# SYSTRAN/faster-whisper

Hardware: AMD Instinct MI355X
Metric: audio-sec/sec (RTF) large-v3 fp16 beam=5 batch=16 (higher is better)
Workload: dtype f16

## Files before the change

### faster_whisper_amd/csrc/attn_enc.hip

```cpp
#include "common.h"
#include "kernels.h"

#define AE_Q 128
#define AE_KV 64
#define AE_VSTRIDE 68
#define AE_LAG 5.0f

__global__ __launch_bounds__(256) void attn_enc_kernel(const half_t* __restrict__ q, const half_t* __restrict__ k,
                                                       int64_t ld, int64_t qk_bstride,
                                                       const half_t* __restrict__ vt, int64_t ldvt,
                                                       int64_t vt_bstride, half_t* __restrict__ out, int64_t ldo,
                                                       int64_t o_bstride, int T, int H, int n_pairs, int n_qt,
                                                       int order) {
  __shared__ __attribute__((aligned(16))) half_t sK[2][AE_KV * 64];
  __shared__ __attribute__((aligned(16))) half_t sV[2][64 * AE_VSTRIDE];

  const int tid = threadIdx.x, lane = tid & 63, wave = tid >> 6;
  const int hi = lane >> 5, l31 = lane & 31;
  const int xcd = blockIdx.x & 7, idx = blockIdx.x >> 3;
  const int pair = order ? (int)blockIdx.x / n_qt : (idx / n_qt) * 8 + xcd;
  if (pair >= n_pairs) return;
  const int b = pair / H, h = pair - b * H, q0 = (order ? (int)blockIdx.x % n_qt : idx % n_qt) * AE_Q;

  const half_t* qb = q + (size_t)b * qk_bstride + h * 64;
  const half_t* kb = k + (size_t)b * qk_bstride + h * 64;
  const half_t* vb = vt + (size_t)b * vt_bstride + (size_t)(h * 64) * ldvt;

  half8_t qf[4];
  {
    int qr = q0 + wave * 32 + l31;
    if (qr > T - 1) qr = T - 1;
    const half_t* qp = qb + (size_t)qr * ld + hi * 8;
#pragma unroll
    for (int ks = 0; ks < 4; ++ks) {
      half8_t v = *reinterpret_cast<const half8_t*>(qp + ks * 16);
#pragma unroll
      for (int e = 0; e < 8; ++e) v[e] = (half_t)((float)v[e] * (0.125f * 1.4426950408889634f));
      qf[ks] = v;
    }
  }

  const int c = tid & 7, r0 = tid >> 3;
  const int nkt = (T + AE_KV - 1) / AE_KV;
  intx4 rk[2], rv[2];
  auto gload = [&](int kt) {
#pragma unroll
    for (int i = 0; i < 2; ++i) {
      const int row = r0 + 32 * i;
      int key = kt * AE_KV + row;
      if (key > T - 1) key = T - 1;
      rk[i] = *reinterpret_cast<const intx4*>(kb + (size_t)key * ld + c * 8);
      rv[i] = *reinterpret_cast<const intx4*>(vb + (size_t)row * ldvt + kt * AE_KV + c * 8);
    }
  };
  auto lstore = [&](int buf) {
#pragma unroll
    for (int i = 0; i < 2; ++i) {
      const int row = r0 + 32 * i;
      *reinterpret_cast<intx4*>(&sK[buf][row * 64 + ((c ^ ((row >> 1) & 7)) << 3)]) = rk[i];
      intx2* dv = reinterpret_cast<intx2*>(&sV[buf][row * AE_VSTRIDE + c * 8]);
      dv[0] = intx2{rv[i][0], rv[i][1]};
      dv[1] = intx2{rv[i][2], rv[i][3]};
    }
  };

  gload(0);
  lstore(0);
  __syncthreads();

  floatx16 o[2] = {floatx16{0}, floatx16{0}};
  floatx16 lsum = floatx16{0};
  const half8_t ones8 = {(half_t)1.f, (half_t)1.f, (half_t)1.f, (half_t)1.f, (half_t)1.f, (half_t)1.f, (half_t)1.f, (half_t)1.f};
  float m_ref = 0.f;
  floatx16 cneg = floatx16{0};

  for (int kt = 0; kt < nkt; ++kt) {
    const int cur = kt & 1;
    const bool more = (kt + 1) < nkt;
    if (more) gload(kt + 1);

    floatx16 s[2];
#pragma unroll
    for (int ks = 0; ks < 4; ++ks) {
      const int chunk = ks * 2 + hi;
#pragma unroll
      for (int kb2 = 0; kb2 < 2; ++kb2) {
        const int row = kb2 * 32 + l31;
        const half8_t kf = *reinterpret_cast<const half8_t*>(&sK[cur][row * 64 + ((chunk ^ ((row >> 1) & 7)) << 3)]);
        s[kb2] = __builtin_amdgcn_mfma_f32_32x32x16_f16(kf, qf[ks], ks == 0 ? cneg : s[kb2], 0, 0, 0);
      }
    }
    const int kbase = kt * AE_KV + 4 * hi;
    const bool tail = (kt * AE_KV + AE_KV) > T;
    if (tail) {
#pragma unroll
      for (int kb2 = 0; kb2 < 2; ++kb2)
#pragma unroll
        for (int r = 0; r < 16; ++r) {
          const int key = kbase + kb2 * 32 + (r & 3) + 8 * (r >> 2);
          if (key >= T) s[kb2][r] = -1.0e30f;
        }
    }
    float mx = fmaxf(s[0][0], s[1][0]);
#pragma unroll
    for (int r = 1; r < 16; ++r) mx = __builtin_fmaxf(__builtin_fmaxf(mx, s[0][r]), s[1][r]);
    mx = pair32_max(mx);
    if (kt == 0 || __builtin_amdgcn_ballot_w64(mx > AE_LAG) != 0) {
      const float delta = kt == 0 ? mx : fmaxf(mx, 0.f);
      const float alpha = kt == 0 ? 1.f : __builtin_amdgcn_exp2f(-delta);
      m_ref += delta;
#pragma unroll
      for (int r = 0; r < 16; ++r) { cneg[r] = -m_ref; lsum[r] *= alpha; }
#pragma unroll
      for (int dt = 0; dt < 2; ++dt)
#pragma unroll
        for (int r = 0; r < 16; ++r) o[dt][r] *= alpha;
#pragma unroll
      for (int kb2 = 0; kb2 < 2; ++kb2)
#pragma unroll
        for (int r = 0; r < 16; ++r) s[kb2][r] -= delta;
    }
#pragma unroll
    for (int kb2 = 0; kb2 < 2; ++kb2)
#pragma unroll
      for (int r = 0; r < 16; ++r) s[kb2][r] = __builtin_amdgcn_exp2f(s[kb2][r]);

#pragma unroll
    for (int kb2 = 0; kb2 < 2; ++kb2)
#pragma unroll
      for (int ks2 = 0; ks2 < 2; ++ks2) {
        half8_t pf;
#pragma unroll
        for (int e = 0; e < 8; e += 2) {
          const half2_t h2 = {(half_t)s[kb2][ks2 * 8 + e], (half_t)s[kb2][ks2 * 8 + e + 1]};
          pf[e] = h2[0]; pf[e + 1] = h2[1];
        }
        lsum = __builtin_amdgcn_mfma_f32_32x32x16_f16(ones8, pf, lsum, 0, 0, 0);
        const int koff = kb2 * 32 + ks2 * 16 + 4 * hi;
#pragma unroll
        for (int dt = 0; dt < 2; ++dt) {
          const half_t* vr = &sV[cur][(dt * 32 + l31) * AE_VSTRIDE + koff];
          const half4_t v0 = *reinterpret_cast<const half4_t*>(vr);
          const half4_t v1 = *reinterpret_cast<const half4_t*>(vr + 8);
          half8_t vf;
#pragma unroll
          for (int e = 0; e < 4; ++e) { vf[e] = v0[e]; vf[4 + e] = v1[e]; }
          o[dt] = __builtin_amdgcn_mfma_f32_32x32x16_f16(vf, pf, o[dt], 0, 0, 0);
        }
      }

    if (more) lstore(cur ^ 1);
    __syncthreads();
  }

  const float inv = 1.0f / lsum[0];
  const int qr = q0 + wave * 32 + l31;
  if (qr < T) {
    half_t* op = out + (size_t)b * o_bstride + (size_t)qr * ldo + h * 64;
#pragma unroll
    for (int dt = 0; dt < 2; ++dt)
#pragma unroll
      for (int g = 0; g < 4; ++g) {
        half4_t ov;
#pragma unroll
        for (int e = 0; e < 4; ++e) ov[e] = (half_t)(o[dt][g * 4 + e] * inv);
        *reinterpret_cast<half4_t*>(op + dt * 32 + 8 * g + 4 * hi) = ov;
      }
  }
}

namespace fwk {
void launch_attn_enc(hipStream_t st, const half_t* q, const half_t* k, int64_t ld, int64_t qk_bstride,
                     const half_t* vt, int64_t ldvt, int64_t vt_bstride, half_t* out, int64_t ldo,
                     int64_t o_bstride, int B, int H, int T, int order) {
  const int n_qt = (T + AE_Q - 1) / AE_Q, n_pairs = B * H;
  const int grid = ((n_pairs + 7) / 8) * 8 * n_qt;
  attn_enc_kernel<<<grid, 256, 0, st>>>(q, k, ld, qk_bstride, vt, ldvt, vt_bstride, out, ldo, o_bstride, T, H, n_pairs, n_qt, order);
}
}
```

### faster_whisper_amd/csrc/engine.hip

```cpp
#include "engine.h"

#include <math.h>
#include <stdarg.h>
#include <stdio.h>
#include <stdlib.h>
#include <string.h>

#include <algorithm>

#include "dec_kernels.h"
#include "kernels.h"

namespace fw {

static thread_local char g_err[1024] = "";
void set_error(const char* fmt, ...) {
  va_list ap;
  va_start(ap, fmt);
  vsnprintf(g_err, sizeof(g_err), fmt, ap);
  va_end(ap);
}

int dev_alloc(void** p, size_t bytes) {
  if (bytes == 0) bytes = 256;
// ... 1499 lines not shown
  {
    std::lock_guard<std::mutex> lk(fm->impl.prof_mu);
    for (auto& p : fm->impl.prof) p = ProfAcc();
  }
  for (Model* l : fm->impl.xlanes) {
    if (!l) continue;
    prof_collect(l);
    std::lock_guard<std::mutex> lk(l->prof_mu);
    for (auto& p : l->prof) p = ProfAcc();
  }
}
int32_t fw_prof_count(void) { return PF_COUNT; }
const char* fw_prof_name(int32_t i) { return (i >= 0 && i < PF_COUNT) ? kProfNames[i] : ""; }
int32_t fw_prof_get(fw_model* fm, int32_t i, double* ms, int64_t* launches, double* flops, double* bytes) {
  FW_CHECK_ARG(fm && i >= 0 && i < PF_COUNT, "bad profile index");
  prof_collect(&fm->impl);
  ProfAcc p;
  {
    std::lock_guard<std::mutex> lk(fm->impl.prof_mu);
    p = fm->impl.prof[i];
  }
  for (Model* l : fm->impl.xlanes) {
    if (!l) continue;
    prof_collect(l);
    std::lock_guard<std::mutex> lk(l->prof_mu);
    p.ms += l->prof[i].ms; p.launches += l->prof[i].launches; p.flops += l->prof[i].flops; p.bytes += l->prof[i].bytes;
  }
  if (ms) *ms = p.ms;
  if (launches) *launches = p.launches;
  if (flops) *flops = p.flops;
  if (bytes) *bytes = p.bytes;
  return FW_OK;
}
int32_t fw_synchronize(fw_model* fm) {
  FW_CHECK_ARG(fm, "null model");
  FW_HIP(hipSetDevice(fm->impl.device));
  FW_HIP(hipStreamSynchronize(fm->impl.stream));
  if (fm->impl.dec_stream) FW_HIP(hipStreamSynchronize(fm->impl.dec_stream));
  for (Model* l : fm->impl.xlanes)
    if (l && l->dec_stream) FW_HIP(hipStreamSynchronize(l->dec_stream));
  return FW_OK;
}
int32_t fw_dev_alloc(fw_model* fm, int64_t bytes, void** out_dev) {
  FW_CHECK_ARG(fm && out_dev && bytes >= 0, "bad argument");
  FW_HIP(hipSetDevice(fm->impl.device));
  return dev_alloc(out_dev, (size_t)bytes);
}
int32_t fw_dev_free(fw_model* fm, void* dev) {
  FW_CHECK_ARG(fm, "null model");
  FW_HIP(hipSetDevice(fm->impl.device));
  if (dev) FW_HIP(hipFree(dev));
  return FW_OK;
}
int32_t fw_dev_upload(fw_model* fm, void* dst_dev, const void* src_host, int64_t bytes) {
  FW_CHECK_ARG(fm && dst_dev && src_host && bytes >= 0, "bad argument");
  FW_HIP(hipSetDevice(fm->impl.device));
  FW_HIP(hipMemcpy(dst_dev, src_host, (size_t)bytes, hipMemcpyHostToDevice));
  return FW_OK;
}

static int upload_f16(Model* m, const float* src, size_t n, half_t** dst) {
  int rc = dev_alloc_t(dst, n);
  if (rc) return rc;
  std::vector<uint16_t> tmp(n);
  for (size_t i = 0; i < n; ++i) tmp[i] = f32_to_f16_bits(src[i]);
  FW_HIP(hipMemcpy(*dst, tmp.data(), n * 2, hipMemcpyHostToDevice));
  return FW_OK;
}
static int download_f16(Model* m, const half_t* src, size_t n, float* dst) {
  std::vector<uint16_t> tmp(n);
  FW_HIP(hipStreamSynchronize(m->stream));
  FW_HIP(hipMemcpy(tmp.data(), src, n * 2, hipMemcpyDeviceToHost));
  for (size_t i = 0; i < n; ++i) {
    half_t h;
    memcpy(&h, &tmp[i], 2);
    dst[i] = (float)h;
  }
  return FW_OK;
}

static inline size_t cross_kv_frag_pos(bool vt, int kvp, int mm, int n) {
  const int c = n & 63, r = mm & 31;
  const size_t head = (size_t)(n >> 6) * kvp * 64;
  return vt ? head + ((size_t)((mm >> 5) * 4 + (c >> 4)) * 64 + ((mm >> 3) & 3) * 16 + (c & 15)) * 8 + (mm & 7)
            : head + ((size_t)((mm >> 5) * 4 + 2 * ((r >> 2) & 1) + (c >> 5)) * 64 + ((c >> 3) & 3) * 16 + (((r >> 3) << 2) | (r & 3))) * 8 + (c & 7);
}

int32_t fw_test_gemm(fw_model* fm, const float* A, const float* W, const float* bias, const float* residual,
                     int32_t M, int32_t N, int32_t K, int32_t act_gelu, int32_t use_int8, float* out) {
  FW_CHECK_ARG(fm && A && W && out, "null argument");
  Model* m = &fm->impl;
  std::lock_guard<std::mutex> lk(m->mu);
  FW_HIP(hipSetDevice(m->device));
  half_t *dA = nullptr, *dW = nullptr, *dB = nullptr, *dR = nullptr, *dC = nullptr;
  int rc;
  if ((rc = upload_f16(m, A, (size_t)M * K, &dA))) return rc;
  if ((rc = upload_f16(m, W, (size_t)N * K, &dW))) return rc;
  if (bias && (rc = upload_f16(m, bias, N, &dB))) return rc;
  if (residual && (rc = upload_f16(m, residual, (size_t)M * N, &dR))) return rc;
  if ((rc = dev_alloc_t(&dC, (size_t)M * N))) return rc;
  LinearW L{dW, dB, nullptr, nullptr, nullptr, nullptr, N, K};
  int8_t* dWq = nullptr;
  float* dWs = nullptr;
  if (use_int8) {
    if (m->compute_type != FW_COMPUTE_INT8_FLOAT16 || (int64_t)M * K > (int64_t)m->max_batch * 1500 * 4 * m->cfg.d_model ||
        M > m->max_batch * 1500) {
      set_error("int8 gemm test needs an int8_float16 model and M*K within its quantisation workspace");
      return FW_EINVAL;
    }
    std::vector<int8_t> wq((size_t)N * K);
    std::vector<float> ws(N);
    for (int n = 0; n < N; ++n) {
      float amax = 0.f;
      for (int k = 0; k < K; ++k) amax = std::max(amax, fabsf(f16_bits_to_f32(f32_to_f16_bits(W[(size_t)n * K + k]))));
      const float sc = amax > 0.f ? 127.0f / amax : 0.f;
      for (int k = 0; k < K; ++k)
        wq[(size_t)n * K + k] = (int8_t)lrintf(f16_bits_to_f32(f32_to_f16_bits(W[(size_t)n * K + k])) * sc);
      ws[n] = amax > 0.f ? amax / 127.0f : 1.0f;
    }
    if ((rc = dev_alloc_t(&dWq, wq.size()))) return rc;
    if ((rc = dev_alloc_t(&dWs, ws.size()))) return rc;
    FW_HIP(hipMemcpy(dWq, wq.data(), wq.size(), hipMemcpyHostToDevice));
    FW_HIP(hipMemcpy(dWs, ws.data(), ws.size() * sizeof(float), hipMemcpyHostToDevice));
    L.wq = dWq; L.wscale = dWs;
    if (act_gelu >= 2)
      rc = run_linear_i8(m, L, dA, nullptr, dC, M, 0, nullptr, 0, 0, M, 1, act_gelu - 2, true, 0);
    else
      rc = run_linear_i8(m, L, dA, nullptr, dC, N, 0, dR, N, 0, M, 1, act_gelu, false, 0);
  } else if (act_gelu == 8 || act_gelu == 9) {
    const bool vt = act_gelu == 9;
    if (N % 64 || residual) { set_error("fragment-major gemm test: N %% 64 == 0, no residual"); return FW_EINVAL; }
    const int kvp = (M + 31) / 32 * 32, H = N / 64;
    half_t* dF = nullptr;
    if ((rc = dev_alloc_t(&dF, (size_t)H * kvp * 64))) return rc;
    FW_HIP(hipMemset(dF, 0, (size_t)H * kvp * 64 * sizeof(half_t)));
    rc = vt ? run_linear(m, L, dA, K, 0, dF, kvp, 0, nullptr, 0, 0, M, 1, 0, true, kvp)
            : run_linear(m, L, dA, K, 0, dF, N, 0, nullptr, 0, 0, M, 1, 0, false, kvp);
    std::vector<float> hf((size_t)H * kvp * 64);
    if (!rc) rc = download_f16(m, dF, hf.size(), hf.data());
    (void)hipFree(dF);
    if (!rc) {
      for (int mm = 0; mm < kvp && !rc; ++mm)
        for (int n = 0; n < N; ++n) {
          const size_t off = cross_kv_frag_pos(vt, kvp, mm, n);
          if (mm < M) out[(size_t)mm * N + n] = hf[off];
          else if (hf[off] != 0.f) { set_error("fragment-major epilogue wrote the padded key %d", mm); rc = FW_ERUNTIME; break; }
        }
    }
    for (half_t* p : {dA, dW, dB, dR, dC})
      if (p) (void)hipFree(p);
    return rc;
  } else if (act_gelu >= 2) {
    rc = run_linear(m, L, dA, K, 0, dC, M, 0, nullptr, 0, 0, M, 1, act_gelu - 2, true);
  } else {
    rc = run_linear(m, L, dA, K, 0, dC, N, 0, dR, N, 0, M, 1, act_gelu, false);
  }
  if (!rc) rc = download_f16(m, dC, (size_t)M * N, out);
  for (half_t* p : {dA, dW, dB, dR, dC})
    if (p) (void)hipFree(p);
  if (dWq) (void)hipFree(dWq);
  if (dWs) (void)hipFree(dWs);
  return rc;
}

static inline size_t frag_pos(int64_t row, int64_t k, int64_t K, int KE) {
  const int OCT = KE / 4;
  return (size_t)((((row >> 4) * (K / KE) + k / KE) * 64 + ((k / OCT) & 3) * 16 + (row & 15)) * OCT + (k % OCT));
}

int32_t fw_test_dec_linear(fw_model* fm, const float* x, const float* W, const float* bias, const float* ln_g,
                           const float* ln_b, const float* res, int32_t R, int32_t N, int32_t K, int32_t act,
                           int32_t use_int8, float* out, float* out_from_frag) {
  FW_CHECK_ARG(fm && x && W && out && out_from_frag, "null argument");
  FW_CHECK_ARG(R >= 1 && N % 32 == 0 && K % 64 == 0, "need R >= 1, N %% 32 == 0, K %% 64 == 0");
  FW_CHECK_ARG((ln_g == nullptr) == (ln_b == nullptr), "ln_g and ln_b go together");
  Model* m = &fm->impl;
  std::lock_guard<std::mutex> lk(m->mu);
  FW_HIP(hipSetDevice(m->device));
  hipStream_t st = m->stream;
  const int R16 = (R + 15) / 16 * 16;
  auto h = [](float v) { return f16_bits_to_f32(f32_to_f16_bits(v)); };
  std::vector<void*> owned;
  auto up = [&](const void* src, size_t bytes, void** dst) -> int {
    int rc = dev_alloc(dst, bytes);
    if (rc) return rc;
    owned.push_back(*dst);
    FW_HIP(hipMemcpy(*dst, src, bytes, hipMemcpyHostToDevice));
    return FW_OK;
  };
  auto cleanup = [&]() { for (void* p : owned) (void)hipFree(p); };
  int rc = FW_OK;
  half_t *d_res = nullptr, *d_bias = nullptr, *d_out = nullptr, *d_of = nullptr;
  std::vector<uint16_t> tmp;
  if (res) {
    tmp.resize((size_t)R * N);
    for (size_t i = 0; i < tmp.size(); ++i) tmp[i] = f32_to_f16_bits(res[i]);
    if ((rc = up(tmp.data(), tmp.size() * 2, (void**)&d_res))) { cleanup(); return rc; }
  }
  if ((rc = dev_alloc_t(&d_out, (size_t)R * N))) { cleanup(); return rc; }
  owned.push_back(d_out);
  if ((rc = dev_alloc_t(&d_of, (size_t)R16 * N))) { cleanup(); return rc; }
  owned.push_back(d_of);
  FW_HIP(hipMemset(d_of, 0, (size_t)R16 * N * 2));
  if (use_int8 == 1) {
    if (m->compute_type != FW_COMPUTE_INT8_FLOAT16 || ln_g) {
      cleanup();
      set_error("int8 decoder-linear test needs an int8_float16 model and no LayerNorm");
      return FW_EINVAL;
    }
    std::vector<int8_t> wq((size_t)N * K);
    std::vector<float> ws(N);
    for (int n = 0; n < N; ++n) {
      float amax = 0.f;
      for (int k = 0; k < K; ++k) amax = std::max(amax, fabsf(h(W[(size_t)n * K + k])));
      const float sc = amax > 0.f ? 127.0f / amax : 0.f;
      for (int k = 0; k < K; ++k) wq[frag_pos(n, k, K, 64)] = (int8_t)lrintf(h(W[(size_t)n * K + k]) * sc);
      ws[n] = amax > 0.f ? amax / 127.0f : 1.0f;
    }
    int8_t *d_wq = nullptr, *d_xq = nullptr;
    float *d_ws = nullptr, *d_xs = nullptr;
    half_t* d_x = nullptr;
    tmp.resize((size_t)R * K);
    for (size_t i = 0; i < tmp.size(); ++i) tmp[i] = f32_to_f16_bits(x[i]);
    if ((rc = up(wq.data(), wq.size(), (void**)&d_wq)) || (rc = up(ws.data(), ws.size() * 4, (void**)&d_ws)) ||
        (rc = up(tmp.data(), tmp.size() * 2, (void**)&d_x))) { cleanup(); return rc; }
    if (bias) {
      tmp.resize(N);
      for (int n = 0; n < N; ++n) tmp[n] = f32_to_f16_bits(bias[n]);
      if ((rc = up(tmp.data(), (size_t)N * 2, (void**)&d_bias))) { cleanup(); return rc; }
    }
    if ((rc = dev_alloc_t(&d_xq, (size_t)R16 * K))) { cleanup(); return rc; }
    owned.push_back(d_xq);
    if ((rc = dev_alloc_t(&d_xs, (size_t)R16))) { cleanup(); return rc; }
    owned.push_back(d_xs);
    FW_HIP(hipMemset(d_xq, 0, (size_t)R16 * K));
    fwk::launch_quant_rows(st, d_x, K, nullptr, nullptr, d_xq, d_xs, R, K, 1);
    if (fwd::launch_dec_gemm_frag_i8(st, d_xq, d_xs, d_wq, d_ws, d_bias, d_res, N, d_out, N, R, N, K, act) != 0) {
      cleanup();
      set_error("int8 decoder linear: unsupported shape R=%d N=%d K=%d", R, N, K);
      return FW_ERUNTIME;
    }
    rc = download_f16(m, d_out, (size_t)R * N, out);
    if (!rc) memcpy(out_from_frag, out, (size_t)R * N * sizeof(float));
    cleanup();
    return rc;
  }
  std::vector<uint16_t> wf((size_t)N * K), xf((size_t)R16 * K, 0);
  std::vector<float> s1(N, 0.f), cf(N, 0.f);
  for (int n = 0; n < N; ++n) {
    double a1 = 0.0, ac = 0.0;
    for (int k = 0; k < K; ++k) {
      const float wv = h(W[(size_t)n * K + k]);
      const uint16_t wg = ln_g ? f32_to_f16_bits(wv * h(ln_g[k])) : f32_to_f16_bits(wv);
      wf[frag_pos(n, k, K, 32)] = wg;
      a1 += (double)f16_bits_to_f32(wg);
      if (ln_g) ac += (double)wv * (double)h(ln_b[k]);
    }
    if (bias) ac += (double)h(bias[n]);
    s1[n] = (float)a1;
    cf[n] = (float)ac;
  }
  for (int r = 0; r < R; ++r)
    for (int k = 0; k < K; ++k) xf[frag_pos(r, k, K, 32)] = f32_to_f16_bits(x[(size_t)r * K + k]);
  half_t *d_wf = nullptr, *d_xf = nullptr;
  float *d_s1 = nullptr, *d_cf = nullptr;
  if ((rc = up(wf.data(), wf.size() * 2, (void**)&d_wf)) || (rc = up(xf.data(), xf.size() * 2, (void**)&d_xf))) {
    cleanup();
    return rc;
  }
  if (ln_g) {
    if ((rc = up(s1.data(), (size_t)N * 4, (void**)&d_s1)) || (rc = up(cf.data(), (size_t)N * 4, (void**)&d_cf))) {
      cleanup();
      return rc;
    }
  } else if (bias) {
    tmp.resize(N);
    for (int n = 0; n < N; ++n) tmp[n] = f32_to_f16_bits(bias[n]);
    if ((rc = up(tmp.data(), (size_t)N * 2, (void**)&d_bias))) { cleanup(); return rc; }
  }
  const int lr =
      use_int8 >= 10 ? fwd::launch_dec_gemm_big(st, use_int8 - 10, d_xf, d_wf, d_bias, d_s1, d_cf, d_res, N, d_out, N, d_of, R, N, K, act)
      : use_int8 == 5 ? fwd::launch_dec_gemm_skinny(st, d_xf, d_wf, d_bias, d_s1, d_cf, d_res, N, d_out, N, d_of, R, N, K, act)
      : (use_int8 == 6 || use_int8 == 7) ? fwd::launch_dec_gemm_skinny_tiles(st, use_int8 - 5, d_xf, d_wf, d_bias, d_s1, d_cf, d_res, N, d_out, N, d_of, R, N, K, act)
                      : fwd::launch_dec_gemm_frag(st, d_xf, d_wf, d_bias, d_s1, d_cf, d_res, N, d_out, N, d_of, R, N, K, act);
  if (lr != 0) {
    cleanup();
    set_error("decoder linear: unsupported shape R=%d N=%d K=%d", R, N, K);
    return FW_ERUNTIME;
  }
  rc = download_f16(m, d_out, (size_t)R * N, out);
  std::vector<float> of((size_t)R16 * N);
  if (!rc) rc = download_f16(m, d_of, (size_t)R16 * N, of.data());
  if (!rc)
    for (int r = 0; r < R; ++r)
      for (int n = 0; n < N; ++n) out_from_frag[(size_t)r * N + n] = of[frag_pos(r, n, N, 32)];
  cleanup();
  return rc;
}

int32_t fw_dec_big_min_rows(void) { return fwd::dec_big_min_rows(); }
int32_t fw_dec_big_min_rows_of(int32_t role, int32_t compute_type) { return fwd::dec_big_min_rows_of(role, compute_type); }

int32_t fw_test_knob(int32_t id, int32_t value) {
  FW_CHECK_ARG(id == 1 || id == 2 || id == 4 || id == 5 || id == 6 || id == 7, "unknown knob %d", id);
  if (id == 6) { set_cross_kv_layered(value); return FW_OK; }
  if (id == 7) { fwd::set_cross_attn_regs(value); return FW_OK; }
  if (id == 1) fwk::g_gemm_order.store(value);
  else if (id == 5) fwk::g_gemm_vt_stage.store(value);
  else if (id == 2) fwd::set_self_attn_form(value);
  else set_pos_blocks(value);
  return FW_OK;
}

int64_t fw_test_idle_lead_chunks(int64_t queued, int32_t n_queued, int32_t encoding, int64_t want, int32_t max_batch) {
  return idle_lead_chunks(queued, n_queued, encoding, want, max_batch);
}

int32_t fw_test_dec_logits(fw_model* fm, const float* x, int32_t R, float* out) {
  FW_CHECK_ARG(fm && x && out && R >= 1, "bad argument");
  Model* m = &fm->impl;
  std::lock_guard<std::mutex> lk(m->mu);
  FW_HIP(hipSetDevice(m->device));
  hipStream_t st = m->stream;
  const int d = m->cfg.d_model, V = m->cfg.n_vocab, R16 = (R + 15) / 16 * 16;
  const bool i8 = m->compute_type == FW_COMPUTE_INT8_FLOAT16;
  std::vector<uint16_t> xh((size_t)R16 * d, 0);
  for (int r = 0; r < R; ++r)
    for (int k = 0; k < d; ++k)
      xh[i8 ? (size_t)r * d + k : frag_pos(r, k, d, 32)] = f32_to_f16_bits(x[(size_t)r * d + k]);
  half_t* d_x = nullptr;
  int8_t* d_xq = nullptr;
  float *d_xs = nullptr, *d_out = nullptr;
  int rc;
  auto cleanup = [&]() { for (void* p : {(void*)d_x, (void*)d_xq, (void*)d_xs, (void*)d_out}) if (p) (void)hipFree(p); };
  if ((rc = dev_alloc_t(&d_x, xh.size())) || (rc = dev_alloc_t(&d_out, (size_t)R * V))) { cleanup(); return rc; }
  FW_HIP(hipMemcpy(d_x, xh.data(), xh.size() * 2, hipMemcpyHostToDevice));
  int lr;
  if (i8) {
    if ((rc = dev_alloc_t(&d_xq, (size_t)R16 * d)) || (rc = dev_alloc_t(&d_xs, (size_t)R16))) { cleanup(); return rc; }
    FW_HIP(hipMemset(d_xq, 0, (size_t)R16 * d));
    fwk::launch_quant_rows(st, d_x, d, m->dec_ln.g, m->dec_ln.b, d_xq, d_xs, R, d, 1);
    lr = fwd::launch_dec_logits(st, true, d_xq, d_xs, m->logits.wq, m->logits.wscale, nullptr, nullptr, d_out, V, R, V, d);
  } else {
    lr = fwd::launch_dec_logits(st, false, d_x, nullptr, m->logits.w, nullptr, m->logits.s1, m->logits.cf, d_out, V, R, V,
                                d);
  }
  hipError_t he = hipSuccess;
  if (lr == 0) he = hipMemcpyAsync(out, d_out, (size_t)R * V * sizeof(float), hipMemcpyDeviceToHost, st);
  if (he == hipSuccess) he = hipStreamSynchronize(st);
  cleanup();
  if (lr != 0 || he != hipSuccess) {
    set_error("logits projection test failed: %s", lr ? "unsupported shape" : hipGetErrorString(he));
    return FW_ERUNTIME;
  }
  return FW_OK;
}

int32_t fw_bench_dec_linear(fw_model* fm, int32_t R, int32_t N, int32_t K, int32_t lnf, int32_t variant, int32_t iters,
                            float* us_out) {
  FW_CHECK_ARG(fm && us_out && R > 0 && N > 0 && K > 0 && iters > 0, "bad argument");
  Model* m = &fm->impl;
  std::lock_guard<std::mutex> lk(m->mu);
  FW_HIP(hipSetDevice(m->device));
  const size_t wn = (size_t)N * K;
  const int copies = (int)std::max<size_t>(2, ((size_t)640 << 20) / (wn * 2));
  const size_t rp = ((size_t)R + 15) / 16 * 16;
  half_t *dW = nullptr, *dX = nullptr, *dO = nullptr, *dB = nullptr;
  float *dS = nullptr, *dC = nullptr;
  int rc;
  auto cleanup = [&]() { for (void* p : {(void*)dW, (void*)dX, (void*)dO, (void*)dB, (void*)dS, (void*)dC}) if (p) (void)hipFree(p); };
  if ((rc = dev_alloc_t(&dW, wn * copies)) || (rc = dev_alloc_t(&dX, rp * K)) || (rc = dev_alloc_t(&dO, rp * N)) ||
      (rc = dev_alloc_t(&dB, (size_t)N)) || (rc = dev_alloc_t(&dS, (size_t)N)) || (rc = dev_alloc_t(&dC, (size_t)N))) {
    cleanup();
    return rc;
  }
  {
    std::vector<uint16_t> h(std::max(wn, rp * (size_t)K));
    uint32_t sd = 2463534242u;
    for (auto& v : h) { sd = sd * 1664525u + 1013904223u; v = f32_to_f16_bits(((int)(sd >> 16) % 2001 - 1000) * 1e-3f); }
    for (int c = 0; c < copies; ++c) FW_HIP(hipMemcpy(dW + (size_t)c * wn, h.data(), wn * 2, hipMemcpyHostToDevice));
    FW_HIP(hipMemcpy(dX, h.data(), rp * K * 2, hipMemcpyHostToDevice));
  }
  FW_HIP(hipMemset(dB, 0, (size_t)N * 2));
  FW_HIP(hipMemset(dS, 0, (size_t)N * 4));
  FW_HIP(hipMemset(dC, 0, (size_t)N * 4));
  hipEvent_t e0, e1;
  FW_HIP(hipEventCreate(&e0));
  FW_HIP(hipEventCreate(&e1));
  hipStream_t st = m->stream;
  int lr = 0;
  for (int i = 0; i < 4 && lr == 0; ++i)
    lr = fwd::launch_dec_gemm_frag_variant(st, variant, lnf != 0, dX, dW + (size_t)(i % copies) * wn, dB, dS, dC, dO, R, N, K);
  FW_HIP(hipEventRecord(e0, st));
  for (int i = 0; i < iters && lr == 0; ++i)
    lr = fwd::launch_dec_gemm_frag_variant(st, variant, lnf != 0, dX, dW + (size_t)(i % copies) * wn, dB, dS, dC, dO, R, N, K);
  FW_HIP(hipEventRecord(e1, st));
  hipError_t he = hipEventSynchronize(e1);
  float ms = 0.f;
  if (he == hipSuccess) he = hipEventElapsedTime(&ms, e0, e1);
  (void)hipEventDestroy(e0);
  (void)hipEventDestroy(e1);
  cleanup();
  if (lr != 0) { set_error("fw_bench_dec_linear: unsupported shape / variant"); return FW_EINVAL; }
  if (he != hipSuccess) { set_error("fw_bench_dec_linear: %s", hipGetErrorString(he)); return FW_ENODEV; }
  *us_out = ms * 1000.f / (float)iters;
  return FW_OK;
}

int32_t fw_bench_gemm(fw_model* fm, int32_t M, int32_t N, int32_t K, int32_t batch, int32_t a_pad, int32_t w_pad,
                      int32_t trans, int32_t iters, float* ms_out) {
  FW_CHECK_ARG(fm && ms_out && M > 0 && N > 0 && K > 0 && batch > 0 && iters > 0, "bad argument");
  Model* m = &fm->impl;
  std::lock_guard<std::mutex> lk(m->mu);
  FW_HIP(hipSetDevice(m->device));
  const bool i8 = m->compute_type == FW_COMPUTE_INT8_FLOAT16;
  const int64_t lda = K + a_pad, ldw = K + w_pad;
  const size_t es = i8 ? 1 : 2;
  const int64_t ldct = (M + 63) / 64 * 64;
  const size_t na = (size_t)batch * M * lda, nw = (size_t)N * ldw,
               nc = trans ? (size_t)batch * N * ldct : (size_t)batch * M * N;
  void *dA = nullptr, *dW = nullptr;
  half_t* dC = nullptr;
  float *dsa = nullptr, *dsw = nullptr;
  int rc;
  auto cleanup = [&]() { for (void* p : {dA, dW, (void*)dC, (void*)dsa, (void*)dsw}) if (p) (void)hipFree(p); };
  if ((rc = dev_alloc(&dA, na * es)) || (rc = dev_alloc(&dW, nw * es)) || (rc = dev_alloc_t(&dC, nc))) { cleanup(); return rc; }
  {
    std::vector<uint16_t> h(std::max(na, nw));
    uint32_t st = 12345u;
    for (auto& v : h) { st = st * 1664525u + 1013904223u; v = f32_to_f16_bits(((int)(st >> 16) % 2001 - 1000) * 1e-3f); }
    FW_HIP(hipMemcpy(dA, h.data(), na * es, hipMemcpyHostToDevice));
    FW_HIP(hipMemcpy(dW, h.data(), nw * es, hipMemcpyHostToDevice));
  }
  if (i8) {
    if ((rc = dev_alloc_t(&dsa, (size_t)batch * M)) || (rc = dev_alloc_t(&dsw, (size_t)N))) { cleanup(); return rc; }
    FW_HIP(hipMemset(dsa, 0, (size_t)batch * M * 4));
    FW_HIP(hipMemset(dsw, 0, (size_t)N * 4));
  }
  fwk::GemmParams p;
  memset(&p, 0, sizeof(p));
  p.A = (const half_t*)dA; p.lda = lda; p.a_bstride = (int64_t)M * lda;
  p.W = (const half_t*)dW; p.ldw = ldw;
  p.C = dC; p.ldc = trans ? ldct : N; p.c_bstride = trans ? (int64_t)N * ldct : (int64_t)M * N;
  p.M = M; p.N = N; p.K = K;
  p.a_scale = dsa; p.as_bstride = M; p.w_scale = dsw;
  hipEvent_t e0, e1;
  FW_HIP(hipEventCreate(&e0));
  FW_HIP(hipEventCreate(&e1));
  int lr = fwk::launch_gemm(m->stream, p, batch, trans != 0);
  FW_HIP(hipEventRecord(e0, m->stream));
  for (int i = 0; i < iters && lr == 0; ++i) lr = fwk::launch_gemm(m->stream, p, batch, trans != 0);
  FW_HIP(hipEventRecord(e1, m->stream));
  hipError_t he = hipEventSynchronize(e1);
  float ms = 0.f;
  if (he == hipSuccess) he = hipEventElapsedTime(&ms, e0, e1);
  (void)hipEventDestroy(e0);
  (void)hipEventDestroy(e1);
  cleanup();
  if (lr != 0 || he != hipSuccess) {
    set_error("gemm bench failed: %s", lr ? "unsupported shape" : hipGetErrorString(he));
    return FW_ERUNTIME;
  }
  *ms_out = ms / (float)iters;
  return FW_OK;
}

static int bench_fill(half_t* dst, size_t n, std::vector<uint16_t>& h, uint32_t seed) {
  if (h.size() < n) h.resize(n);
  for (size_t i = 0; i < n; ++i) { seed = seed * 1664525u + 1013904223u; h[i] = f32_to_f16_bits(((int)(seed >> 16) % 2001 - 1000) * 1e-3f); }
  FW_HIP(hipMemcpy(dst, h.data(), n * 2, hipMemcpyHostToDevice));
  return FW_OK;
}

int32_t fw_bench_gemm_epi(fw_model* fm, int32_t M, int32_t N, int32_t K, int32_t batch, int32_t lda_in, int32_t trans,
                          int32_t bias, int32_t act, int32_t res, int32_t n_layers, int32_t iters, float* ms_out) {
  FW_CHECK_ARG(fm && ms_out && M > 0 && N > 0 && K > 0 && batch > 0 && iters > 0 && n_layers >= 1, "bad argument");
  FW_CHECK_ARG(res >= 0 && res <= 2 && !(res && (trans || n_layers > 1)), "residual: row-major single-layer output only");
  Model* m = &fm->impl;
  FW_CHECK_ARG(m->compute_type != FW_COMPUTE_INT8_FLOAT16, "float16 models only");
  std::lock_guard<std::mutex> lk(m->mu);
  FW_HIP(hipSetDevice(m->device));
  const int64_t lda = lda_in > 0 ? lda_in : K;
  const bool layered = n_layers > 1;
  const int64_t kvp = (M + 31) / 32 * 32;
  const int64_t ldct = layered ? kvp : (M + 63) / 64 * 64;
  const int64_t c_bs = layered ? (int64_t)N * kvp : (trans ? (int64_t)N * ldct : (int64_t)M * N);
  const int64_t c_ls = c_bs * batch;
  const size_t na = (size_t)batch * ((size_t)M * lda + K), nw = (size_t)N * K * n_layers, nc = (size_t)c_ls * n_layers;
  const size_t nr1 = res == 1 ? (size_t)batch * M * N : (size_t)M * N;
  const int copies = res == 1 ? (int)std::max<size_t>(2, ((size_t)640 << 20) / (nr1 * 2)) : 1;
  half_t *dA = nullptr, *dW = nullptr, *dC = nullptr, *dB = nullptr, *dR = nullptr;
  int rc;
  auto cleanup = [&]() { for (void* p : {(void*)dA, (void*)dW, (void*)dC, (void*)dB, (void*)dR}) if (p) (void)hipFree(p); };
  if ((rc = dev_alloc_t(&dA, na)) || (rc = dev_alloc_t(&dW, nw)) || (rc = dev_alloc_t(&dC, nc)) ||
      (rc = dev_alloc_t(&dB, (size_t)N * n_layers)) || (res && (rc = dev_alloc_t(&dR, nr1 * copies)))) {
    cleanup();
    return rc;
  }
  {
    std::vector<uint16_t> h;
    if ((rc = bench_fill(dA, na, h, 12345u)) || (rc = bench_fill(dW, nw, h, 12345u)) ||
        (rc = bench_fill(dB, (size_t)N * n_layers, h, 777u))) { cleanup(); return rc; }
    if (res) {
      if ((rc = bench_fill(dR, nr1, h, 4242u))) { cleanup(); return rc; }
      for (int c = 1; c < copies; ++c) FW_HIP(hipMemcpy(dR + (size_t)c * nr1, dR, nr1 * 2, hipMemcpyDeviceToDevice));
    }
    FW_HIP(hipMemset(dC, 0, nc * 2));
  }
  fwk::GemmParams p;
  memset(&p, 0, sizeof(p));
  p.A = dA; p.lda = lda; p.a_bstride = (int64_t)M * lda;
  p.W = dW; p.ldw = K;
  p.bias = bias ? dB : nullptr;
  p.C = dC; p.ldc = layered ? (trans ? kvp : N) : (trans ? ldct : N); p.c_bstride = c_bs;
  p.M = M; p.N = N; p.K = K;
  p.act = act;
  if (layered) {
    p.head_rows = (int)kvp;
    p.n_layers = n_layers; p.w_lstride = (int64_t)N * K; p.bias_lstride = N; p.c_lstride = c_ls;
  }
  p.ldr = N; p.r_bstride = res == 1 ? (int64_t)M * N : 0;
  hipEvent_t e0, e1;
  FW_HIP(hipEventCreate(&e0));
  FW_HIP(hipEventCreate(&e1));
  p.res = dR;
  int lr = fwk::launch_gemm(m->stream, p, batch, trans != 0);
  FW_HIP(hipEventRecord(e0, m->stream));
  for (int i = 0; i < iters && lr == 0; ++i) {
    if (res) p.res = dR + (size_t)(i % copies) * nr1;
    lr = fwk::launch_gemm(m->stream, p, batch, trans != 0);
  }
  FW_HIP(hipEventRecord(e1, m->stream));
  hipError_t he = hipEventSynchronize(e1);
  float ms = 0.f;
  if (he == hipSuccess) he = hipEventElapsedTime(&ms, e0, e1);
  (void)hipEventDestroy(e0);
  (void)hipEventDestroy(e1);
  cleanup();
  if (lr != 0 || he != hipSuccess) {
    set_error("gemm epilogue bench failed: %s", lr ? "unsupported shape" : hipGetErrorString(he));
    return FW_ERUNTIME;
  }
  *ms_out = ms / (float)iters;
  return FW_OK;
}

int32_t fw_bench_dec_linear_epi(fw_model* fm, int32_t R, int32_t N, int32_t K, int32_t lnf, int32_t variant, int32_t act,
                                int32_t res, int32_t outs, int32_t iters, float* us_out) {
  FW_CHECK_ARG(fm && us_out && R > 0 && N > 0 && K > 0 && iters > 0, "bad argument");
  FW_CHECK_ARG((outs & 3) != 0 && (!res || (outs & 1)), "needs an output; the residual is the row-major output in place");
  FW_CHECK_ARG(variant == 0 || variant == 5 || (variant >= 10 && variant <= 12), "unknown variant %d", variant);
  Model* m = &fm->impl;
  std::lock_guard<std::mutex> lk(m->mu);
  FW_HIP(hipSetDevice(m->device));
  const size_t wn = (size_t)N * K;
  const int copies = (int)std::max<size_t>(2, ((size_t)640 << 20) / (wn * 2));
  const size_t rp = ((size_t)R + 15) / 16 * 16, on = rp * N;
  const int ocopies = (int)std::max<size_t>(2, ((size_t)640 << 20) / (on * 2));
  half_t *dW = nullptr, *dX = nullptr, *dO = nullptr, *dF = nullptr, *dB = nullptr;
  float *dS = nullptr, *dC = nullptr;
  int rc;
  auto cleanup = [&]() { for (void* p : {(void*)dW, (void*)dX, (void*)dO, (void*)dF, (void*)dB, (void*)dS, (void*)dC}) if (p) (void)hipFree(p); };
  if ((rc = dev_alloc_t(&dW, wn * copies)) || (rc = dev_alloc_t(&dX, rp * K)) || (rc = dev_alloc_t(&dO, on * ocopies)) ||
      (rc = dev_alloc_t(&dF, on)) || (rc = dev_alloc_t(&dB, (size_t)N)) || (rc = dev_alloc_t(&dS, (size_t)N)) ||
      (rc = dev_alloc_t(&dC, (size_t)N))) {
    cleanup();
    return rc;
  }
  {
    std::vector<uint16_t> h;
    if ((rc = bench_fill(dW, wn, h, 2463534242u)) || (rc = bench_fill(dX, rp * K, h, 2463534242u))) { cleanup(); return rc; }
    for (int c = 1; c < copies; ++c) FW_HIP(hipMemcpy(dW + (size_t)c * wn, dW, wn * 2, hipMemcpyDeviceToDevice));
  }
  FW_HIP(hipMemset(dO, 0, on * ocopies * 2));
  FW_HIP(hipMemset(dB, 0, (size_t)N * 2));
  FW_HIP(hipMemset(dS, 0, (size_t)N * 4));
  FW_HIP(hipMemset(dC, 0, (size_t)N * 4));
  hipEvent_t e0, e1;
  FW_HIP(hipEventCreate(&e0));
  FW_HIP(hipEventCreate(&e1));
  hipStream_t st = m->stream;
  auto go = [&](int i) -> int {
    const half_t* w = dW + (size_t)(i % copies) * wn;
    half_t* o = dO + (size_t)(i % ocopies) * on;
    half_t* op = (outs & 1) ? o : nullptr;
    half_t* of = (outs & 2) ? dF : nullptr;
    const half_t* r = res ? o : nullptr;
    const half_t* b = lnf ? nullptr : dB;
    const float *s1 = lnf ? dS : nullptr, *cf = lnf ? dC : nullptr;
    if (variant >= 10) return fwd::launch_dec_gemm_big(st, variant - 10, dX, w, b, s1, cf, r, N, op, N, of, R, N, K, act);
    if (variant == 5) return fwd::launch_dec_gemm_skinny(st, dX, w, b, s1, cf, r, N, op, N, of, R, N, K, act);
    return fwd::launch_dec_gemm_frag(st, dX, w, b, s1, cf, r, N, op, N, of, R, N, K, act);
  };
  int lr = 0;
  for (int i = 0; i < 4 && lr == 0; ++i) lr = go(i);
  FW_HIP(hipEventRecord(e0, st));
  for (int i = 0; i < iters && lr == 0; ++i) lr = go(i);
  FW_HIP(hipEventRecord(e1, st));
  hipError_t he = hipEventSynchronize(e1);
  float ms = 0.f;
  if (he == hipSuccess) he = hipEventElapsedTime(&ms, e0, e1);
  (void)hipEventDestroy(e0);
  (void)hipEventDestroy(e1);
  cleanup();
  if (lr != 0) { set_error("fw_bench_dec_linear_epi: unsupported shape / variant"); return FW_EINVAL; }
  if (he != hipSuccess) { set_error("fw_bench_dec_linear_epi: %s", hipGetErrorString(he)); return FW_ENODEV; }
  *us_out = ms * 1000.f / (float)iters;
// ... 262 lines not shown
```

### faster_whisper_amd/csrc/kernels.h

```cpp
#pragma once
#include <atomic>
#include "common.h"

namespace fwk {

size_t logmel_lds_bytes();
void launch_logmel(hipStream_t st, const float* pcm_dev, const int64_t* offsets_dev, int B, int max_frames_total,
                   const float* consts, const float* filtT, int mel_pad, int n_mels, float* raw,
                   int64_t raw_bstride, int raw_stride, int* chunk_max, int drop_last, int out_frames,
                   float* out_f32, half_t* out_cl, int c_pad, int* n_frames_out);
void launch_features_to_cl(hipStream_t st, const float* feats_dev, int B, int n_mels, int frames, half_t* out_cl,
                           int c_pad);

struct GemmParams {
  const half_t* A; int64_t lda; int64_t a_bstride;
  const half_t* W; int64_t ldw;
  const half_t* bias;
  const half_t* res; int64_t ldr; int64_t r_bstride;
  half_t* C; int64_t ldc; int64_t c_bstride;
  int M, N, K;
  int act;
  int head_rows;
  const float* a_scale; int64_t as_bstride; const float* w_scale;
  int nMt, nNt;
  int n_mp, blk_m, blk_n;
  int vt_stage;
  int n_layers; int64_t w_lstride, bias_lstride, c_lstride;
  int nNt_layer;
};
int launch_gemm(hipStream_t st, const GemmParams& p, int batch, bool trans);
extern std::atomic<int> g_gemm_order;
extern std::atomic<int> g_gemm_vt_stage;

void launch_layernorm(hipStream_t st, const half_t* x, const half_t* g, const half_t* b, half_t* y, int rows, int d,
                      int frag = 0);
void launch_quant_rows(hipStream_t st, const half_t* x, int64_t ldx, const half_t* g, const half_t* b, int8_t* xq,
                       float* scale, int rows, int d, int frag = 0);
void launch_f32_to_f16(hipStream_t st, const float* x, half_t* y, int64_t n);
void launch_f16_to_f32(hipStream_t st, const half_t* x, float* y, int64_t n);

void launch_attn_enc(hipStream_t st, const half_t* q, const half_t* k, int64_t ld, int64_t qk_bstride,
                     const half_t* vt, int64_t ldvt, int64_t vt_bstride, half_t* out, int64_t ldo,
                     int64_t o_bstride, int B, int H, int T, int order = 0);

}
```

### profiles/attn_bench.py

```python
import ctypes as C
import os
import sys

sys.path.insert(0, os.path.dirname(os.path.dirname(os.path.abspath(__file__))))
from faster_whisper_amd import Whisper, _lib, get_config, synthetic_weights


def main():
    cfg = get_config("micro")
    m = Whisper("synthetic:micro", device="cuda", files={"config": cfg, "weights": synthetic_weights(cfg, seed=1)},
                max_batch_size=1, max_beam_size=1)
    h = m._replicas[0].handle
    ms = C.c_float()
    B, H, T = 16, 20, 1500
    fl = 4.0 * B * H * T * T * 64
    only = int(sys.argv[1]) if len(sys.argv) > 1 else -1
    for rnd in range(3):
        for variant, what in ((0, "XCD-aware grid"), (1, "round-3 grid")):
            if only >= 0 and variant != only:
                continue
            _lib.check(m._lib.fw_bench_attention(h, B, H, T, variant, 50, C.byref(ms)))
            print(f"round {rnd} {what}: {ms.value * 1e3:.1f} us per launch, {fl / ms.value / 1e9:.0f} TFLOP/s", flush=True)


if __name__ == "__main__":
    main()
```

Before: 3184.

## Software-pipeline encoder attention tile loop with prefetched LDS fragments and peeled tail

Adds a new default form of the encoder flash-attention kernel. It restructures the KV tile loop: K and V fragments are prefetched from LDS ahead of their MFMAs, and sched_group_barrier hints interleave the LDS reads with the matrix ops. Global loads use precomputed 32-bit offsets with pointer bumping, and the last two tiles are peeled so steady-state iterations skip the clamping and tail-masking checks. The goal is to hide LDS and global latency and cut per-iteration address arithmetic, at the cost of higher register pressure and more complex code. The old loop stays available through a knob and as a fallback when strides are too wide for 32-bit offsets.

Measured after the change: 3207 (median of 5 runs). About the same (+0.7%).

```diff
diff --git a/faster_whisper_amd/csrc/attn_enc.hip b/faster_whisper_amd/csrc/attn_enc.hip
--- a/faster_whisper_amd/csrc/attn_enc.hip
+++ b/faster_whisper_amd/csrc/attn_enc.hip
@@ -1,11 +1,14 @@
 #include "common.h"
 #include "kernels.h"
+
+#include <type_traits>
 
 #define AE_Q 128
 #define AE_KV 64
 #define AE_VSTRIDE 68
 #define AE_LAG 5.0f
 
+template <int FORM>
 __global__ __launch_bounds__(256) void attn_enc_kernel(const half_t* __restrict__ q, const half_t* __restrict__ k,
                                                        int64_t ld, int64_t qk_bstride,
                                                        const half_t* __restrict__ vt, int64_t ldvt,
@@ -15,8 +18,9 @@
   __shared__ __attribute__((aligned(16))) half_t sK[2][AE_KV * 64];
   __shared__ __attribute__((aligned(16))) half_t sV[2][64 * AE_VSTRIDE];
 
-  const int tid = threadIdx.x, lane = tid & 63, wave = tid >> 6;
-  const int hi = lane >> 5, l31 = lane & 31;
+  const int tid = threadIdx.x;
+  int lane = tid & 63, wave = tid >> 6;
+  int hi = lane >> 5, l31 = lane & 31;
   const int xcd = blockIdx.x & 7, idx = blockIdx.x >> 3;
   const int pair = order ? (int)blockIdx.x / n_qt : (idx / n_qt) * 8 + xcd;
   if (pair >= n_pairs) return;
@@ -40,7 +44,7 @@
     }
   }
 
-  const int c = tid & 7, r0 = tid >> 3;
+  int c = tid & 7, r0 = tid >> 3;
   const int nkt = (T + AE_KV - 1) / AE_KV;
   intx4 rk[2], rv[2];
   auto gload = [&](int kt) {
@@ -74,6 +78,153 @@
   float m_ref = 0.f;
   floatx16 cneg = floatx16{0};
 
+  if constexpr (FORM == 0) {
+  const char* ktile = reinterpret_cast<const char*>(kb + (size_t)AE_KV * ld);
+  const char* vtile = reinterpret_cast<const char*>(vb + AE_KV);
+  uint32_t koff[2], voff[2];
+#pragma unroll
+  for (int i = 0; i < 2; ++i) {
+    koff[i] = (uint32_t)(r0 + 32 * i) * (uint32_t)ld * 2u + c * 16;
+    voff[i] = (uint32_t)(r0 + 32 * i) * (uint32_t)ldvt * 2u + c * 16;
+  }
+  const size_t kstep = (size_t)AE_KV * ld * 2;
+  auto gnext = [&]() {
+#pragma unroll
+    for (int i = 0; i < 2; ++i) {
+      asm volatile("" : "+v"(koff[i]), "+v"(voff[i]));
+      rk[i] = *reinterpret_cast<const intx4*>(ktile + koff[i]);
+      rv[i] = *reinterpret_cast<const intx4*>(vtile + voff[i]);
+    }
+    ktile += kstep;
+    vtile += AE_KV * 2;
+  };
+  const int ka0 = l31 * 128 + ((hi ^ ((l31 >> 1) & 7)) << 4);
+  const int lk0 = r0 * 64 + ((c ^ ((r0 >> 1) & 7)) << 3), lv0 = r0 * AE_VSTRIDE + c * 8;
+  auto tile = [&](const int kt, auto next_c) {
+    constexpr int NEXT = decltype(next_c)::value;
+    const int cur = kt & 1;
+    if constexpr (NEXT == 1) gnext();
+    if constexpr (NEXT == 2) gload(kt + 1);
+
+    floatx16 s[2];
+    const int ka = cur * (AE_KV * 128) + ka0;
+    auto kfrag = [&](int ks, int kb2) {
+      return *reinterpret_cast<const half8_t*>(reinterpret_cast<const char*>(&sK[0][0]) + ((ka ^ (ks * 32)) + kb2 * 32 * 128));
+    };
+    half8_t kf[4][2];
+    kf[0][0] = kfrag(0, 0); kf[0][1] = kfrag(0, 1);
+    kf[1][0] = kfrag(1, 0); kf[1][1] = kfrag(1, 1);
+    __builtin_amdgcn_sched_group_barrier(0x100, 4, 0);
+    const half_t* sVc = &sV[cur][l31 * AE_VSTRIDE + 4 * hi];
+    auto vfrag = [&](int sl, int dt) {
+      const half_t* vr = sVc + dt * 32 * AE_VSTRIDE + sl * 16;
+      const half4_t v0 = *reinterpret_cast<const half4_t*>(vr);
+      const half4_t v1 = *reinterpret_cast<const half4_t*>(vr + 8);
+      half8_t vf;
+#pragma unroll
+      for (int e = 0; e < 4; ++e) { vf[e] = v0[e]; vf[4 + e] = v1[e]; }
+      return vf;
+    };
+    half8_t vf[4][2];
+#pragma unroll
+    for (int ks = 0; ks < 4; ++ks) {
+      if (ks + 2 < 4) { kf[ks + 2][0] = kfrag(ks + 2, 0); kf[ks + 2][1] = kfrag(ks + 2, 1); }
+      else if (ks == 2) { vf[0][0] = vfrag(0, 0); vf[0][1] = vfrag(0, 1); }
+#pragma unroll
+      for (int kb2 = 0; kb2 < 2; ++kb2)
+        s[kb2] = __builtin_amdgcn_mfma_f32_32x32x16_f16(kf[ks][kb2], qf[ks], ks == 0 ? cneg : s[kb2], 0, 0, 0);
+      if (ks == 0) asm volatile("" :: "v"(cneg));
+      __builtin_amdgcn_sched_group_barrier(0x008, 2, 0);
+      if (ks < 3) __builtin_amdgcn_sched_group_barrier(0x100, 2, 0);
+    }
+    if constexpr (NEXT == 0) {
+      const int kbase = kt * AE_KV + 4 * hi;
+      if ((kt * AE_KV + AE_KV) > T) {
+#pragma unroll
+        for (int kb2 = 0; kb2 < 2; ++kb2)
+#pragma unroll
+          for (int r = 0; r < 16; ++r) {
+            const int key = kbase + kb2 * 32 + (r & 3) + 8 * (r >> 2);
+            if (key >= T) s[kb2][r] = -1.0e30f;
+          }
+      }
+    }
+    float mc[4];
+#pragma unroll
+    for (int kb2 = 0; kb2 < 2; ++kb2) {
+      const floatx16& a = s[kb2];
+      float m = __builtin_fmaxf(__builtin_fmaxf(a[0], a[1]), a[2]);
+      m = __builtin_fmaxf(__builtin_fmaxf(m, a[3]), a[4]);
+      mc[kb2 * 2] = __builtin_fmaxf(__builtin_fmaxf(m, a[5]), a[6]);
+      m = __builtin_fmaxf(__builtin_fmaxf(a[7], a[8]), a[9]);
+      m = __builtin_fmaxf(__builtin_fmaxf(m, a[10]), a[11]);
+      m = __builtin_fmaxf(__builtin_fmaxf(m, a[12]), a[13]);
+      mc[kb2 * 2 + 1] = __builtin_fmaxf(__builtin_fmaxf(m, a[14]), a[15]);
+    }
+    float mx = __builtin_fmaxf(__builtin_fmaxf(__builtin_fmaxf(mc[0], mc[1]), mc[2]), mc[3]);
+    mx = pair32_max(mx);
+    if (kt == 0 || __builtin_amdgcn_ballot_w64(mx > AE_LAG) != 0) {
+      const float delta = kt == 0 ? mx : fmaxf(mx, 0.f);
+      const float alpha = kt == 0 ? 1.f : __builtin_amdgcn_exp2f(-delta);
+      m_ref += delta;
+#pragma unroll
+      for (int r = 0; r < 16; ++r) { cneg[r] = -m_ref; lsum[r] *= alpha; }
+#pragma unroll
+      for (int dt = 0; dt < 2; ++dt)
+#pragma unroll
+        for (int r = 0; r < 16; ++r) o[dt][r] *= alpha;
+#pragma unroll
+      for (int kb2 = 0; kb2 < 2; ++kb2)
+#pragma unroll
+        for (int r = 0; r < 16; ++r) s[kb2][r] -= delta;
+    }
+#pragma unroll
+    for (int kb2 = 0; kb2 < 2; ++kb2)
+#pragma unroll
+      for (int r = 0; r < 16; ++r) s[kb2][r] = __builtin_amdgcn_exp2f(s[kb2][r]);
+
+#pragma unroll
+    for (int kb2 = 0; kb2 < 2; ++kb2)
+#pragma unroll
+      for (int ks2 = 0; ks2 < 2; ++ks2) {
+        half8_t pf;
+#pragma unroll
+        for (int e = 0; e < 8; e += 2) {
+          const half2_t h2 = {(half_t)s[kb2][ks2 * 8 + e], (half_t)s[kb2][ks2 * 8 + e + 1]};
+          pf[e] = h2[0]; pf[e + 1] = h2[1];
+        }
+        lsum = __builtin_amdgcn_mfma_f32_32x32x16_f16(ones8, pf, lsum, 0, 0, 0);
+        const int sl = kb2 * 2 + ks2;
+        if (sl + 1 < 4) { vf[sl + 1][0] = vfrag(sl + 1, 0); vf[sl + 1][1] = vfrag(sl + 1, 1); }
+#pragma unroll
+        for (int dt = 0; dt < 2; ++dt) o[dt] = __builtin_amdgcn_mfma_f32_32x32x16_f16(vf[sl][dt], pf, o[dt], 0, 0, 0);
+        if (sl + 1 < 4) __builtin_amdgcn_sched_group_barrier(0x100, 2, 0);
+        __builtin_amdgcn_sched_group_barrier(0x008, 3, 0);
+      }
+
+    if constexpr (NEXT != 0) {
+      half_t* dk = &sK[0][(cur ^ 1) * (AE_KV * 64) + lk0];
+      half_t* dv = &sV[0][(cur ^ 1) * (64 * AE_VSTRIDE) + lv0];
+#pragma unroll
+      for (int i = 0; i < 2; ++i) {
+        *reinterpret_cast<intx4*>(dk + i * 32 * 64) = rk[i];
+        intx2* d2 = reinterpret_cast<intx2*>(dv + i * 32 * AE_VSTRIDE);
+        d2[0] = intx2{rv[i][0], rv[i][1]};
+        d2[1] = intx2{rv[i][2], rv[i][3]};
+      }
+    }
+    __syncthreads();
+  };
+  int kt = 0;
+  for (; kt + 2 < nkt; ++kt) tile(kt, std::integral_constant<int, 1>{});
+  {
+    int t2 = tid;
+    asm volatile("" : "+v"(t2));
+    lane = t2 & 63; wave = t2 >> 6; hi = lane >> 5; l31 = lane & 31; c = t2 & 7; r0 = t2 >> 3;
+  }
+  if (kt + 1 < nkt) { tile(kt, std::integral_constant<int, 2>{}); ++kt; }
+  tile(kt, std::integral_constant<int, 0>{});
+  } else {
   for (int kt = 0; kt < nkt; ++kt) {
     const int cur = kt & 1;
     const bool more = (kt + 1) < nkt;
@@ -152,6 +303,7 @@
     if (more) lstore(cur ^ 1);
     __syncthreads();
   }
+  }
 
   const float inv = 1.0f / lsum[0];
   const int qr = q0 + wave * 32 + l31;
@@ -170,11 +322,16 @@
 }
 
 namespace fwk {
+std::atomic<int> g_attn_enc_form{0};
 void launch_attn_enc(hipStream_t st, const half_t* q, const half_t* k, int64_t ld, int64_t qk_bstride,
                      const half_t* vt, int64_t ldvt, int64_t vt_bstride, half_t* out, int64_t ldo,
                      int64_t o_bstride, int B, int H, int T, int order) {
   const int n_qt = (T + AE_Q - 1) / AE_Q, n_pairs = B * H;
   const int grid = ((n_pairs + 7) / 8) * 8 * n_qt;
-  attn_enc_kernel<<<grid, 256, 0, st>>>(q, k, ld, qk_bstride, vt, ldvt, vt_bstride, out, ldo, o_bstride, T, H, n_pairs, n_qt, order);
+  const bool wide = (uint64_t)ld * AE_KV * 2 >= (1ull << 32) || (uint64_t)ldvt * AE_KV * 2 >= (1ull << 32);
+  if (g_attn_enc_form.load() == 1 || wide)
+    attn_enc_kernel<1><<<grid, 256, 0, st>>>(q, k, ld, qk_bstride, vt, ldvt, vt_bstride, out, ldo, o_bstride, T, H, n_pairs, n_qt, order);
+  else
+    attn_enc_kernel<0><<<grid, 256, 0, st>>>(q, k, ld, qk_bstride, vt, ldvt, vt_bstride, out, ldo, o_bstride, T, H, n_pairs, n_qt, order);
 }
 }
diff --git a/faster_whisper_amd/csrc/engine.hip b/faster_whisper_amd/csrc/engine.hip
--- a/faster_whisper_amd/csrc/engine.hip
+++ b/faster_whisper_amd/csrc/engine.hip
@@ -1825,7 +1825,8 @@
 int32_t fw_dec_big_min_rows_of(int32_t role, int32_t compute_type) { return fwd::dec_big_min_rows_of(role, compute_type); }
 
 int32_t fw_test_knob(int32_t id, int32_t value) {
-  FW_CHECK_ARG(id == 1 || id == 2 || id == 4 || id == 5 || id == 6 || id == 7, "unknown knob %d", id);
+  FW_CHECK_ARG(id == 1 || id == 2 || id == 4 || id == 5 || id == 6 || id == 7 || id == 8, "unknown knob %d", id);
+  if (id == 8) { fwk::g_attn_enc_form.store(value); return FW_OK; }
   if (id == 6) { set_cross_kv_layered(value); return FW_OK; }
   if (id == 7) { fwd::set_cross_attn_regs(value); return FW_OK; }
   if (id == 1) fwk::g_gemm_order.store(value);
diff --git a/faster_whisper_amd/csrc/kernels.h b/faster_whisper_amd/csrc/kernels.h
--- a/faster_whisper_amd/csrc/kernels.h
+++ b/faster_whisper_amd/csrc/kernels.h
@@ -39,6 +39,7 @@
 void launch_f32_to_f16(hipStream_t st, const float* x, half_t* y, int64_t n);
 void launch_f16_to_f32(hipStream_t st, const half_t* x, float* y, int64_t n);
 
+extern std::atomic<int> g_attn_enc_form;
 void launch_attn_enc(hipStream_t st, const half_t* q, const half_t* k, int64_t ld, int64_t qk_bstride,
                      const half_t* vt, int64_t ldvt, int64_t vt_bstride, half_t* out, int64_t ldo,
                      int64_t o_bstride, int B, int H, int T, int order = 0);
diff --git a/profiles/attn_bench.py b/profiles/attn_bench.py
--- a/profiles/attn_bench.py
+++ b/profiles/attn_bench.py
@@ -15,12 +15,16 @@
     B, H, T = 16, 20, 1500
     fl = 4.0 * B * H * T * T * 64
     only = int(sys.argv[1]) if len(sys.argv) > 1 else -1
-    for rnd in range(3):
-        for variant, what in ((0, "XCD-aware grid"), (1, "round-3 grid")):
-            if only >= 0 and variant != only:
-                continue
-            _lib.check(m._lib.fw_bench_attention(h, B, H, T, variant, 50, C.byref(ms)))
-            print(f"round {rnd} {what}: {ms.value * 1e3:.1f} us per launch, {fl / ms.value / 1e9:.0f} TFLOP/s", flush=True)
+    try:
+        for rnd in range(3):
+            for form, what in ((1, "tile loop of rounds 4-7"), (0, "tile loop of round 8")):
+                if only >= 0 and form != only:
+                    continue
+                _lib.check(m._lib.fw_test_knob(8, form))
+                _lib.check(m._lib.fw_bench_attention(h, B, H, T, 0, 50, C.byref(ms)))
+                print(f"round {rnd} {what}: {ms.value * 1e3:.1f} us per launch, {fl / ms.value / 1e9:.0f} TFLOP/s", flush=True)
+    finally:
+        _lib.check(m._lib.fw_test_knob(8, 0))
 
 
 if __name__ == "__main__":
```
